# akanimax/thr3ed_atom

Measured on AMD Instinct MI355X. Metric: ray-samples/sec (fwd+bwd) training step, 800x800 images @ 128^3 SH-2 ReLU field, higher is better.
Workload: dtype f32

## Files before the change

### thr3ed_atom_amd/csrc/relu_field_kernels.hip

```cpp
#include "rf_device.h"

#include <atomic>

namespace {

#ifndef RF_FWD_WAVES
#define RF_FWD_WAVES 4
#endif
#ifndef RF_EMIT_WAVES
#define RF_EMIT_WAVES 6
#endif
#ifndef RF_EMIT_G
#define RF_EMIT_G 2
#endif
constexpr short kNoBrick = -1;

struct __attribute__((packed, aligned(4))) f4u {
  float v[4];
};
struct __attribute__((packed, aligned(4))) f3u {
  float v[3];
};
typedef float vf2 __attribute__((ext_vector_type(2)));
typedef float vf4 __attribute__((ext_vector_type(4)));
// ... 411 lines not shown
      }
      if (!L::kCorner && g.layout == RF_LAYOUT_SPLIT) {
        if constexpr (!L::kCorner) {
          const float rest = rest_colour_sums<K>(prod);
          if (has && ls.closes_colour) my_rgb[slot * 4 + ls.colour] = rest;
        }
      } else {
#pragma unroll
        for (int ch = 0; ch < 3; ++ch) rgb[ch] = group_sum_to_last<LPS>(rgb[ch]);
        if (has && sub == LPS - 1) {
          if constexpr (L::kCorner) {
#pragma unroll
            for (int ch = 0; ch < 3; ++ch) rgb[ch] = kC0 * rgb[ch];
          }
          my_rgb[slot * 4 + 0] = rgb[0];
          my_rgb[slot * 4 + 1] = rgb[1];
          my_rgb[slot * 4 + 2] = rgb[2];
        }
      }
    }
    wave_lds_fence();

    const float raw_r = fast_base ? fast_rgb[0] : (base_in_p0 ? fast_rgb[0] + my_rgb[slot * 4 + 0] : my_rgb[slot * 4 + 0]);
    const float raw_g = fast_base ? fast_rgb[1] : (base_in_p0 ? fast_rgb[1] + my_rgb[slot * 4 + 1] : my_rgb[slot * 4 + 1]);
    const float raw_b = fast_base ? fast_rgb[2] : (base_in_p0 ? fast_rgb[2] + my_rgb[slot * 4 + 2] : my_rgb[slot * 4 + 2]);
    if (need) {
      part_c[0] += w * sigmoidf_(raw_r);
      part_c[1] += w * sigmoidf_(raw_g);
      part_c[2] += w * sigmoidf_(raw_b);
    }
    if (sm.valid) {
      part_acc += w;
      part_depth += w * sm.z;
    }
    if constexpr (SAVE) {
      if (need) {
        const long long idx = ray * (long long)r.S + chunk * kWave + slot;
        float4 cv;
        cv.x = raw_r;
        cv.y = raw_g;
        cv.z = raw_b;
        cv.w = sigma;
        store_f4<RF_NT_CACHE_STORE>(reinterpret_cast<float4*>(out.cache) + idx, cv);
        if (RF_NT_CACHE_STORE)
          __builtin_nontemporal_store(T, out.tcache + idx);
        else
          out.tcache[idx] = T;
      }
      my_cmask = (lane == (chunk & (kWave - 1))) ? mask : my_cmask;
      if (out.hist) add_key_runs<false>(out.hist, need ? brick_key(sm.cell.i0, g, out.brick_shift, out.nby, out.nbz) : -1, lane);
    }
    wave_lds_fence();
    if (T_carry == 0.0f) break;
  }

  const float cr = wave_sum(part_c[0]), cg = wave_sum(part_c[1]), cb = wave_sum(part_c[2]);
  const float acc = wave_sum(part_acc), depth = wave_sum(part_depth);
  if (lane == 0) {
    const float bg = white ? (1.0f - acc) : 0.0f;
    out.colour[ray * 3 + 0] = white ? cr + bg : cr;
    out.colour[ray * 3 + 1] = white ? cg + bg : cg;
    out.colour[ray * 3 + 2] = white ? cb + bg : cb;
    out.depth[ray] = depth;
    out.acc[ray] = acc;
    const float q = depth / acc;
    out.disparity[ray] = 1.0f / ((q != q) ? q : fmaxf(kZeroPlus, q));
    if constexpr (SAVE) out.stop[ray] = processed;
  }
  if constexpr (SAVE) {
    flush_cmasks(cmask_group);
    for (int gq = cmask_group + 1; gq * kWave < nchunks; ++gq) flush_cmasks(gq);
  }
}

template <int K, bool DIFFUSE, bool SAVE>
__global__ __launch_bounds__(kBlock, RF_FWD_WAVES) void render_forward_kernel(GridArgs g, RayArgs r, OutArgs out, uint32_t flags) {
  __shared__ __attribute__((aligned(16))) uint32_t s_entry[kWavesPerBlock][kWave * kEntryFwd];
  __shared__ __attribute__((aligned(16))) float s_rgb[kWavesPerBlock][kWave * 4];
  const int lane = threadIdx.x & (kWave - 1);
  const int wave = __builtin_amdgcn_readfirstlane(threadIdx.x >> 6);
  render_forward_ray<K, DIFFUSE, SAVE>(g, r, out, flags, (long long)blockIdx.x * kWavesPerBlock + wave, lane, s_entry[wave], s_rgb[wave]);
}

struct ForwardPair {
  RayArgs r[2];
  OutArgs out[2];
  uint32_t flags[2];
};
__device__ __forceinline__ void fold_step_switches(GridArgs& g, RayArgs& r, uint32_t& flags) {
  g.layout = RF_LAYOUT_SPLIT;
  g.bricked = 0;
  g.near32 = 1;
  g.mode = RF_DENSITY_RELU;
  g.occ = nullptr;
  g.step[2] = 1u;
#pragma unroll
  for (int a = 0; a < 3; ++a) g.jump[a] = g.step[a];
  r.trand = nullptr;
  r.jitter = 1;
  r.cam = 0;
  r.H = r.W = 1;
  r.focal = 1.0f;
#pragma unroll
  for (int i = 0; i < 12; ++i) r.pose[i] = 0.0f;
  flags &= ~(uint32_t)(RF_FLAG_OCCUPANCY_SKIP | RF_FLAG_AABB_SAMPLING);
}

template <int K, bool DIFFUSE, bool STEP>
__device__ __forceinline__ void forward_pair_ray(const GridArgs& g, const RayArgs& r, const OutArgs& out, uint32_t flags, long long ray, int lane,
                                                 uint32_t* my_entry, float* my_rgb) {
  if constexpr (STEP) {
    GridArgs gl = g;
    RayArgs rl = r;
    fold_step_switches(gl, rl, flags);
    render_forward_ray<K, DIFFUSE, true>(gl, rl, out, flags, ray, lane, my_entry, my_rgb);
  } else {
    render_forward_ray<K, DIFFUSE, true>(g, r, out, flags, ray, lane, my_entry, my_rgb);
  }
}

template <int K, bool STEP>
__global__ __launch_bounds__(kBlock, RF_FWD_WAVES) void render_forward_pair_kernel(GridArgs g, ForwardPair p) {
  __shared__ __attribute__((aligned(16))) uint32_t s_entry[kWavesPerBlock][kWave * kEntryFwd];
  __shared__ __attribute__((aligned(16))) float s_rgb[kWavesPerBlock][kWave * 4];
  const int lane = threadIdx.x & (kWave - 1);
  const int wave = __builtin_amdgcn_readfirstlane(threadIdx.x >> 6);
  const long long ray = (long long)blockIdx.x * (kWavesPerBlock / 2) + (wave & 1);
  if (wave < 2) {
    if constexpr (K == 1)
      forward_pair_ray<1, true, STEP>(g, p.r[0], p.out[0], p.flags[0], ray, lane, s_entry[wave], s_rgb[wave]);
    else
      forward_pair_ray<K, false, STEP>(g, p.r[0], p.out[0], p.flags[0], ray, lane, s_entry[wave], s_rgb[wave]);
  } else {
    forward_pair_ray<1, true, STEP>(g, p.r[1], p.out[1], p.flags[1], ray, lane, s_entry[wave], s_rgb[wave]);
  }
}

#ifndef RF_TILE_WAVES
#define RF_TILE_WAVES 4
#endif
constexpr int kTileXS = 18;
constexpr int kTileSlots = (3 * kTileXS + 16 + 3) / 4 * 4;
#define RF_TILE_SLOT(lane) ((lane) + ((lane) >> 4) * (kTileXS - 16))
struct TileCell {
  int c0[3], e[3];
  float w[8];
};
__device__ __forceinline__ TileCell tile_cell(const Cell& c, const GridArgs& g) {
  const int dims3[3] = {g.X, g.Y, g.Z};
  TileCell t;
  float aw[3][2];
#pragma unroll
  for (int a = 0; a < 3; ++a) {
    const int i0 = c.i0[a];
    const bool ok0 = i0 >= 0, ok1 = i0 + 1 < dims3[a];
    t.c0[a] = max(i0, 0);
    t.e[a] = (ok0 && ok1) ? 1 : 0;
    aw[a][0] = ok0 ? c.w0[a] : 0.0f;
    aw[a][1] = ok1 ? c.w1[a] : 0.0f;
  }
  const float wxy[4] = {aw[0][0] * aw[1][0], aw[0][1] * aw[1][0], aw[0][0] * aw[1][1], aw[0][1] * aw[1][1]};
#pragma unroll
  for (int k = 0; k < 8; ++k) t.w[k] = wxy[k & 3] * aw[2][k >> 2];
  return t;
}

__device__ __forceinline__ void tile_window_origin(bool pending, unsigned long long pm, const int c0[3], int O[3]) {
  const int anchor = ((pm >> 27) & 1ull) ? 27 : __builtin_ctzll(pm);
#pragma unroll
  for (int a = 0; a < 3; ++a) {
    const int A = __builtin_amdgcn_readlane(c0[a], anchor);
    const bool below1 = __ballot(pending && c0[a] < A) != 0ull, below2 = __ballot(pending && c0[a] < A - 1) != 0ull;
    O[a] = A - (below1 ? 1 : 0) - (below2 ? 1 : 0);
  }
}

struct TileWindow {
  vf4 b, q0, q1, q2, q3, q4, q5;
};
__device__ __forceinline__ unsigned int tile_window_node(const GridArgs& g, const int O[3], int lane) {
  const int nx = min(O[0] + (lane >> 4), g.X - 1), ny = min(O[1] + ((lane >> 2) & 3), g.Y - 1), nz = min(O[2] + (lane & 3), g.Z - 1);
  return node_lin(g, nx, ny, nz);
}
__device__ __forceinline__ const char* tile_record(const float* tensor, long long stride, unsigned int lin, int near32) {
  if (near32) return reinterpret_cast<const char*>(tensor) + (size_t)__umul24(lin, (unsigned int)stride * 4u);
  return reinterpret_cast<const char*>(tensor + (size_t)lin * (size_t)stride);
}
__device__ __forceinline__ void tile_window_load_base(TileWindow& wdw, const GridArgs& g, unsigned int lin) {
  wdw.b = *reinterpret_cast<const vf4*>(tile_record(g.dens, g.dstride, lin, g.near32));
}
__device__ __forceinline__ void tile_window_load_rest(TileWindow& wdw, const GridArgs& g, unsigned int lin) {
  const char* rp = tile_record(g.feat, g.fstride, lin, g.near32);
  wdw.q0 = *reinterpret_cast<const vf4*>(rp);
  wdw.q1 = *reinterpret_cast<const vf4*>(rp + 16);
  wdw.q2 = *reinterpret_cast<const vf4*>(rp + 32);
  wdw.q3 = *reinterpret_cast<const vf4*>(rp + 48);
  wdw.q4 = *reinterpret_cast<const vf4*>(rp + 64);
  wdw.q5 = *reinterpret_cast<const vf4*>(rp + 80);
}
__device__ __forceinline__ void tile_window_store_rest(const TileWindow& wdw, vf4* my_rest, int lane) {
  vf4* d = my_rest + RF_TILE_SLOT(lane) * 6;
  d[0] = wdw.q0;
  d[1] = wdw.q1;
  d[2] = wdw.q2;
  d[3] = wdw.q3;
  d[4] = wdw.q4;
  d[5] = wdw.q5;
}

__device__ __forceinline__ bool tile_interpolate_base(bool pending, const TileCell& tc, const int O[3], const vf4* my_base, const GridArgs& g, float T, int nk[8],
                                                      float& sigma, float raw[3], bool& need) {
// ... 597 lines not shown
      dl[u] = sm.delta;
      ix[u][0] = sm.cell.idx[0];
      ix[u][1] = sm.cell.idx[1];
      ix[u][2] = sm.cell.idx[2];
      counted[u] = (cm[u] >> lane) & 1ull;
      const int key = counted[u] ? brick_key(sm.cell.i0, g, gr.brick_shift, gr.nby, gr.nbz) : -1;
      const bool active = key >= 0;
      const int prev = __shfl_up(key, 1);
      const bool head = active && (lane == 0 || prev != key);
      const unsigned long long heads = __ballot(head);
      const unsigned long long ends = __ballot(head || !active);
      const unsigned long long above = (lane == 63) ? 0ull : (ends & ~((2ull << lane) - 1ull));
      const int run = (above ? __builtin_ctzll(above) : 64) - lane;
      const unsigned long long below = heads & ((lane == 63) ? ~0ull : ((2ull << lane) - 1ull));
      hl_[u] = below ? 63 - __builtin_clzll(below) : 0;
      if (head) base_[u] = atomicAdd(&gr.cursor[key], run);
    }
#pragma unroll
    for (int u = 0; u < G; ++u) {
      if (cm[u] == 0ull) continue;
      const bool have = counted[u];
      const float sigma = have ? cv[u].w : 0.0f;
      const float T = have ? Tc[u] : 0.0f;
      float E;
      const float alpha = occupancy_alpha(sigma * dl[u], E);
      const float w = alpha * T;
      const float Tn = T * E;
      const float raw[3] = {cv[u].x, cv[u].y, cv[u].z};
      float c[3], e = gD * zz[u] + gA;
#pragma unroll
      for (int ch = 0; ch < 3; ++ch) {
        c[ch] = sigmoidf_(raw[ch]);
        e += gC[ch] * (c[ch] - white);
      }
      const float we = have ? w * e : 0.0f;
      const float incl = wave_incl_rscan_add(we, lane);
      const float after = (incl - we) + suffix;
      suffix += __shfl(incl, 0, kWave);
      const float g_sigma = dl[u] * (Tn * e - after);
      float g_pre = density_pre_grad(g_sigma, sigma, g.mode);
      const int pos = __shfl(base_[u], hl_[u]) + (lane - hl_[u]);
      if (have) {
        const float graw[3] = {(w * gC[0]) * (c[0] * (1.0f - c[0])), (w * gC[1]) * (c[1] * (1.0f - c[1])), (w * gC[2]) * (c[2] * (1.0f - c[2]))};
        float4* dst = gr.sorted + (long long)pos * QE;
        if constexpr (KE == 1) {
          store_f4<RF_NT_RECORD_STORE>(dst + 0, make_float4(ix[u][0], ix[u][1], ix[u][2], 0.0f));
          store_f4<RF_NT_RECORD_STORE>(dst + 1, make_float4(g_pre * g.rho, graw[0] * kC0, graw[1] * kC0, graw[2] * kC0));
        } else {
          store_f4<RF_NT_RECORD_STORE>(dst + 0, make_float4(ix[u][0], ix[u][1], ix[u][2], g_pre * g.rho));
          store_f4<RF_NT_RECORD_STORE>(dst + 1, make_float4(graw[0], graw[1], graw[2], vdir[0]));
          store_f4<RF_NT_RECORD_STORE>(dst + 2, make_float4(vdir[1], vdir[2], 0.0f, 0.0f));
        }
      }
    }
  }
}

template <int K, bool DIFFUSE>
__global__ __launch_bounds__(kBlock, RF_EMIT_WAVES) void render_emit_direct_kernel(GridArgs g, RayArgs r, OutArgs fwd, GradArgs gr, uint32_t flags) {
  const int lane = threadIdx.x & (kWave - 1);
  const int wave = __builtin_amdgcn_readfirstlane(threadIdx.x >> 6);
  render_emit_direct_ray<K, DIFFUSE>(g, r, fwd, gr, flags, (long long)blockIdx.x * kWavesPerBlock + wave, lane);
}

struct EmitPair {
  RayArgs r[2];
  OutArgs fwd[2];
  GradArgs gr[2];
  uint32_t flags[2];
};
template <int K, bool DIFFUSE, bool STEP>
__device__ __forceinline__ void emit_pair_ray(const GridArgs& g, const RayArgs& r, const OutArgs& fwd, const GradArgs& gr, uint32_t flags, long long ray, int lane) {
  if constexpr (STEP) {
    GridArgs gl = g;
    RayArgs rl = r;
    fold_step_switches(gl, rl, flags);
    render_emit_direct_ray<K, DIFFUSE>(gl, rl, fwd, gr, flags, ray, lane);
  } else {
    render_emit_direct_ray<K, DIFFUSE>(g, r, fwd, gr, flags, ray, lane);
  }
}

template <int K, bool STEP>
__global__ __launch_bounds__(kBlock, RF_EMIT_WAVES) void render_emit_direct_pair_kernel(GridArgs g, EmitPair p) {
  const int lane = threadIdx.x & (kWave - 1);
  const int wave = __builtin_amdgcn_readfirstlane(threadIdx.x >> 6);
  const long long ray = (long long)blockIdx.x * (kWavesPerBlock / 2) + (wave & 1);
  for (int i = 0; i < 2; ++i)
    if (p.gr[i].hist_clear)
      for (long long k = (long long)blockIdx.x * blockDim.x + threadIdx.x; k < p.gr[i].nkeys; k += (long long)gridDim.x * blockDim.x) p.gr[i].hist_clear[k] = 0;
  GradArgs gr = p.gr[wave < 2 ? 0 : 1];
  gr.hist_clear = nullptr;
  if (wave < 2) {
    if constexpr (K == 1)
      emit_pair_ray<1, true, STEP>(g, p.r[0], p.fwd[0], gr, p.flags[0], ray, lane);
    else
      emit_pair_ray<K, false, STEP>(g, p.r[0], p.fwd[0], gr, p.flags[0], ray, lane);
  } else {
    emit_pair_ray<1, true, STEP>(g, p.r[1], p.fwd[1], gr, p.flags[1], ray, lane);
  }
}

constexpr int kMaxListsPerKind = 8;
constexpr int kRangeEntries = 15;
constexpr int kMaxRangesKind = kRangeEntries * kMaxListsPerKind;

struct BrickList {
  const float4* rec;
  const long long* offsets;
};

__device__ __forceinline__ void adam_update(float& p, float& m, float& v, float g, float step, float b1, float b2, float eps,
                                            float inv_bc2_sqrt) {
  const float mm = m + (g - m) * (1.0f - b1);
  const float vv = v * b2 + (g * g) * (1.0f - b2);
  const float denom = __builtin_amdgcn_sqrtf(vv) * inv_bc2_sqrt + eps;
  p = p - step * (mm * __builtin_amdgcn_rcpf(denom));
  m = mm;
  v = vv;
}

struct AdamArgs {
  float* p1;
  float* p2;
  float* m1;
  float* m2;
  float* v1;
  float* v2;
  float step;
  float b1, b2, eps;
  float inv_bc2_sqrt;
  int byte_offsets_fit_32_bits;
};

struct BrickArgs {
  BrickList wide[kMaxListsPerKind];
  BrickList narrow[kMaxListsPerKind];
  int nwide, nnarrow;
  int shift;
  int nbx, nby, nbz;
  int brick_first;
  int accumulate;
  int fmul;
  int stagger;
  AdamArgs adam;
  int parts;
  float* partial;
  int* part_state;
};

template <int Q>
__global__ void expand_records_kernel(const float4* __restrict__ rec, const long long* __restrict__ perm,
                                      const long long* __restrict__ begin_ptr, long long capacity, float4* __restrict__ out) {
  const long long begin = *begin_ptr;
  const long long items = (capacity - begin) * Q;
  for (long long it = (long long)blockIdx.x * blockDim.x + threadIdx.x; it < items; it += (long long)gridDim.x * blockDim.x) {
    const long long i = begin + it / Q;
    const int part = (int)(it % Q);
    out[i * Q + part] = rec[perm[i] * Q + part];
  }
}

struct BinLists {
  const int* hist[2];
  long long* offsets[2];
  int* cursor[2];
};

__device__ __forceinline__ void bin_offsets_body(const BinLists& lists, int nkeys, int list, int block) {
  const int* __restrict__ hist = lists.hist[list];
  long long* __restrict__ offsets = lists.offsets[list];
  int* __restrict__ cursor = lists.cursor[list];
  __shared__ int s_front[16], s_own[16];
  const int t = threadIdx.x, lane = t & (kWave - 1), wave = t >> 6;
  const int seg0 = block * 1024;
  int front = 0;
// ... 1127 lines not shown
    if (ZERO_GRAD) gradp[i] = 0.0f;
  }
}

struct L1Sets {
  const float* colour[2];
  float* grad[2];
  float* sums[2];
};

__device__ __forceinline__ void l1_loss_grad_body(const L1Sets& sets, const float* __restrict__ target, long long n3, float gscale, int set,
                                                  int block, int nblocks) {
  const float* __restrict__ colour = sets.colour[set];
  float* __restrict__ grad = sets.grad[set];
  float* __restrict__ sums = sets.sums[set];
  float abs_sum = 0.0f, sq_sum = 0.0f;
  for (long long i = (long long)block * blockDim.x + threadIdx.x; i < n3; i += (long long)nblocks * blockDim.x) {
    const float d = colour[i] - target[i];
    abs_sum += fabsf(d);
    sq_sum += d * d;
    grad[i] = (d > 0.0f) ? gscale : ((d < 0.0f) ? -gscale : 0.0f);
  }
  __shared__ float s_part[2][16];
  abs_sum = wave_sum(abs_sum);
  sq_sum = wave_sum(sq_sum);
  const int wave = threadIdx.x >> 6;
  if ((threadIdx.x & (kWave - 1)) == 0) {
    s_part[0][wave] = abs_sum;
    s_part[1][wave] = sq_sum;
  }
  __syncthreads();
  if (threadIdx.x == 0) {
    float a = 0.0f, b = 0.0f;
    for (int w = 0; w < (int)(blockDim.x >> 6); ++w) {
      a += s_part[0][w];
      b += s_part[1][w];
    }
    unsafeAtomicAdd(sums + 0, a);
    unsafeAtomicAdd(sums + 1, b);
  }
}

__global__ void l1_loss_grad_kernel(L1Sets sets, const float* __restrict__ target, long long n3, float gscale) {
  l1_loss_grad_body(sets, target, n3, gscale, blockIdx.y, blockIdx.x, gridDim.x);
}

__global__ void l1_loss_pair_kernel(L1Sets sets, const float* __restrict__ target, long long n3, float gscale, float inv_n3, float* __restrict__ out) {
  l1_loss_grad_body(sets, target, n3, gscale, blockIdx.y, blockIdx.x, gridDim.x);
  if (threadIdx.x == 0) {
    float* ws = sets.sums[0];
    unsigned int* ticket = reinterpret_cast<unsigned int*>(ws + 4);
    __threadfence();
    const unsigned int total = gridDim.x * gridDim.y;
    if (atomicAdd(ticket, 1u) == total - 1u) {
      __threadfence();
      float v[4];
#pragma unroll
      for (int i = 0; i < 4; ++i) v[i] = atomicExch(ws + i, 0.0f);
      atomicExch(ticket, 0u);
      const float l0 = v[0] * inv_n3, l1 = v[2] * inv_n3;
      out[0] = l0 + l1;
      out[1] = l0;
      out[2] = v[1] * inv_n3;
      out[3] = l1;
      out[4] = v[3] * inv_n3;
    }
  }
}

__global__ __launch_bounds__(1024) void loss_and_offsets_kernel(L1Sets sets, const float* __restrict__ target, long long n3, float gscale,
                                                                int loss_blocks, BinLists lists, int nkeys, int offset_blocks, int passes) {
  if (!((passes >> (blockIdx.y & 1)) & 1)) return;
  if (blockIdx.y < 2) {
    if ((int)blockIdx.x < loss_blocks) l1_loss_grad_body(sets, target, n3, gscale, blockIdx.y, blockIdx.x, loss_blocks);
  } else if ((int)blockIdx.x < offset_blocks) {
    bin_offsets_body(lists, nkeys, blockIdx.y - 2, blockIdx.x);
  }
}

}

extern "C" {

#ifdef RF_BRICK_PROFILE
int rf_debug_brick_profile(unsigned long long* out_host, int reset) {
  if (hipDeviceSynchronize() != hipSuccess) return RF_ERR_LAUNCH;
  if (out_host && hipMemcpyFromSymbol(out_host, HIP_SYMBOL(g_brick_prof), sizeof(g_brick_prof)) != hipSuccess) return RF_ERR_LAUNCH;
  if (reset) {
    unsigned long long zero[8] = {};
    if (hipMemcpyToSymbol(HIP_SYMBOL(g_brick_prof), zero, sizeof(zero)) != hipSuccess) return RF_ERR_LAUNCH;
  }
  return RF_OK;
}
#endif

int rf_abi_version(void) { return RF_ABI_VERSION; }

int rf_abi_struct_size(int which) {
  switch (which) {
    case 0: return (int)sizeof(RFGrid);
    case 1: return (int)sizeof(RFRayBatch);
    case 2: return (int)sizeof(RFRenderOut);
    case 3: return (int)sizeof(RFRenderGrads);
    case 4: return (int)sizeof(RFBrickList);
    case 5: return (int)sizeof(RFAdamState);
    case 6: return (int)sizeof(RFCamera);
    case 7: return (int)sizeof(RFRaySelection);
    case 8: return (int)sizeof(RFPassScratch);
    case 9: return (int)sizeof(RFTrainStep);
    case 10: return (int)sizeof(RFGeometryOut);
    case 11: return (int)sizeof(RFImage);
    default: return -1;
  }
}

const char* rf_error_string(int code) {
  switch (code) {
    case RF_OK:
      return "ok";
    case RF_ERR_NULL_POINTER:
      return "null pointer";
    case RF_ERR_BAD_SHAPE:
      return "bad shape, size or stride";
    case RF_ERR_UNSUPPORTED:
      return "unsupported configuration (SH degree must be 0..3, density mode a RF_DENSITY_* value, brick size 4 or 8 -- 8 for SH degree 3 -- with at most 4096 bricks for 16-bit keys; the optimizer in the brick flush needs split storage and SH degree 0 or 2)";
    case RF_ERR_LAUNCH:
      return "HIP kernel launch failed";
    default:
      return "unknown error code";
  }
}

int rf_cast_rays(int32_t height, int32_t width, float focal, const float* rotation_host, const float* translation_host,
                 float* origins_dev, float* directions_dev, void* stream) {
  if (!rotation_host || !translation_host || !origins_dev || !directions_dev) return RF_ERR_NULL_POINTER;
  if (height < 1 || width < 1) return RF_ERR_BAD_SHAPE;
  Pose pose;
  for (int i = 0; i < 9; ++i) pose.r[i] = rotation_host[i];
  for (int i = 0; i < 3; ++i) pose.t[i] = translation_host[i];
  const long long n = (long long)height * width;
  hipLaunchKernelGGL(cast_rays_kernel, dim3(grid_1d(n, 256)), dim3(256), 0, (hipStream_t)stream, height, width, focal,
                     pose, origins_dev, directions_dev);
  return launch_status();
}

int rf_cast_selected_rays(int32_t height, int32_t width, float focal, const float* poses_dev, int32_t num_poses,
                          const int64_t* pixel_index_dev, int64_t num_rays, float* origins_dev, float* directions_dev,
                          void* stream) {
  if (num_rays == 0) return RF_OK;
  if (!poses_dev || !pixel_index_dev || !origins_dev || !directions_dev) return RF_ERR_NULL_POINTER;
  if (height < 1 || width < 1 || num_poses < 1 || num_rays < 0) return RF_ERR_BAD_SHAPE;
  hipLaunchKernelGGL(cast_selected_rays_kernel, dim3(grid_1d(num_rays, 256)), dim3(256), 0, (hipStream_t)stream, height,
                     width, focal, poses_dev, num_poses, pixel_index_dev, (long long)num_rays, origins_dev,
                     directions_dev);
  return launch_status();
}

static int select_impl(int32_t height, int32_t width, float focal, const float* poses_dev, const int64_t* image_ids_dev,
                       int32_t num_batch_images, const float* pixel_table_dev, uint64_t key, int64_t first_index, int64_t num_rays,
                       float* origins_dev, float* directions_dev, float* pixels_dev, int64_t* pixel_index_dev, float* zero4_dev,
                       void* stream) {
  if (num_rays == 0) return RF_OK;
  if (!poses_dev || !pixel_table_dev || !origins_dev || !directions_dev || !pixels_dev) return RF_ERR_NULL_POINTER;
  if (height < 1 || width < 1 || num_batch_images < 1 || num_rays < 0 || first_index < 0) return RF_ERR_BAD_SHAPE;
  const unsigned long long P = (unsigned long long)num_batch_images * height * width;
  if ((unsigned long long)(first_index + num_rays) > P) return RF_ERR_BAD_SHAPE;
// ... 122 lines not shown
  }
  const unsigned blocks = ray_blocks(rays->num_rays);
  hipStream_t st = (hipStream_t)stream;
  const bool diffuse = flags & RF_FLAG_RENDER_DIFFUSE;
  const int K = grid->num_features / 3;
  if (rays->camera && !save) {
    const bool tiles = !rays->t_rand_dev && rays->num_samples <= kTileMaxSamples && frame_uses_packets(grid, g, rays->camera, flags);
    if (tiles) {
      const int W = rays->camera->width;
      const int row0 = (int)(rays->first_ray / W), row1 = (int)((rays->first_ray + rays->num_rays - 1) / W);
      const int tile_rows = (row1 - row0) / 8 + 1, tiles_x = (W + 7) / 8;
      static const int wpb = env_int("RF_TILE_WPB", 1) == 4 ? 4 : 1;
      static const bool xcd_rows = env_flag("RF_TILE_XCD_ROWS", true);
      const int KT = diffuse ? 1 : K;
      auto launch = [&](auto k, auto waves, auto xr) {
        constexpr int WPB = decltype(waves)::value;
        const long long wgs = decltype(xr)::value ? (long long)((tile_rows + 7) / 8) * 8 * ((tiles_x + WPB - 1) / WPB) : ((long long)tile_rows * tiles_x + WPB - 1) / WPB;
        hipLaunchKernelGGL((render_frame_tile_kernel<decltype(k)::value, WPB, decltype(xr)::value>), dim3((unsigned)wgs), dim3(kWave * WPB), 0, st, g, r, o, flags, row0, tile_rows, tiles_x);
        return launch_status();
      };
      using One = std::integral_constant<int, 1>;
      using Four = std::integral_constant<int, 4>;
      if (KT == 4 || KT == 16)
        return dispatch_sh(KT, ShSet<4, 16>{}, [&](auto k) { return launch(k, One{}, std::true_type{}); });
      return dispatch_sh(KT, ShSet<9, 1>{}, [&](auto k) {
        if (wpb == 4) return xcd_rows ? launch(k, Four{}, std::true_type{}) : launch(k, Four{}, std::false_type{});
        return xcd_rows ? launch(k, One{}, std::true_type{}) : launch(k, One{}, std::false_type{});
      });
    }
  }
  return dispatch_render(K, diffuse, [&](auto k, auto d) {
    if (save)
      hipLaunchKernelGGL((render_forward_kernel<decltype(k)::value, decltype(d)::value, true>), dim3(blocks), dim3(kBlock), 0, st, g, r, o, flags);
    else
      hipLaunchKernelGGL((render_forward_kernel<decltype(k)::value, decltype(d)::value, false>), dim3(blocks), dim3(kBlock), 0, st, g, r, o, flags);
    return launch_status();
  });
}

static bool step_pair_specialised(const RFGrid* grid, const GridArgs& g, const RFRayBatch* const rays[2], const uint32_t flags[2]) {
  if (!(grid->layout == RF_LAYOUT_SPLIT && g.layout == RF_LAYOUT_SPLIT && !g.bricked && g.near32 && grid->density_mode == RF_DENSITY_RELU)) return false;
  for (int i = 0; i < 2; ++i) {
    if (rays[i]->camera || rays[i]->t_rand_dev || !(flags[i] & RF_FLAG_JITTER_KEYED)) return false;
    if (flags[i] & (RF_FLAG_OCCUPANCY_SKIP | RF_FLAG_AABB_SAMPLING)) return false;
  }
  return env_flag("RF_STEP_SPECIALISED", true);
}

int rf_step_kernel_specialised(const RFGrid* grid, const RFRayBatch* rays, const uint32_t* flags) {
  int rc = check_grid(grid);
  if (rc != RF_OK) return rc;
  if (!rays || !flags) return RF_ERR_NULL_POINTER;
  const RFRayBatch* const rr[2] = {&rays[0], &rays[1]};
  for (int i = 0; i < 2; ++i) {
    rc = check_rays(rr[i]);
    if (rc != RF_OK) return rc;
  }
  if (!renders_pair_up(rr, flags)) return RF_ERR_UNSUPPORTED;
  return step_pair_specialised(grid, to_args(grid), rr, flags) ? 1 : 0;
}

static int forward_pair_impl(const RFGrid* grid, const RFRayBatch* const rays[2], const uint32_t flags[2], const RFRenderOut* const outs[2], void* stream) {
  int rc = check_grid(grid);
  if (rc != RF_OK) return rc;
  ForwardPair p;
  for (int i = 0; i < 2; ++i) {
    rc = check_rays(rays[i]);
    if (rc != RF_OK) return rc;
    const RFRenderOut* out = outs[i];
    if (!out || !out->colour_dev || !out->depth_dev || !out->acc_dev || !out->disparity_dev) return RF_ERR_NULL_POINTER;
    if (!has_caches(out)) return RF_ERR_UNSUPPORTED;
    if ((flags[i] & RF_FLAG_OCCUPANCY_SKIP) && !grid->occupancy_dev) return RF_ERR_NULL_POINTER;
    p.r[i] = to_args(rays[i], flags[i]);
    p.out[i] = to_args(out);
    p.flags[i] = flags[i];
    if (out->key_hist_dev) {
      rc = set_key_hist(grid, out, &p.out[i]);
      if (rc != RF_OK) return rc;
    }
  }
  if (!renders_pair_up(rays, flags)) return RF_ERR_UNSUPPORTED;
  if (rays[0]->num_rays == 0) return RF_OK;
  const GridArgs g = to_args(grid);
  const unsigned blocks = (unsigned)((rays[0]->num_rays + 1) / 2);
  const bool specialised = step_pair_specialised(grid, g, rays, flags);
  return dispatch_sh(grid->num_features / 3, ShAll{}, [&](auto k) {
    if (specialised)
      hipLaunchKernelGGL((render_forward_pair_kernel<decltype(k)::value, true>), dim3(blocks), dim3(kBlock), 0, (hipStream_t)stream, g, p);
    else
      hipLaunchKernelGGL((render_forward_pair_kernel<decltype(k)::value, false>), dim3(blocks), dim3(kBlock), 0, (hipStream_t)stream, g, p);
    return launch_status();
  });
}

static int backward_impl(const RFGrid* grid, const RFRayBatch* rays, uint32_t flags, const RFRenderOut* fwd,
                         const RFRenderGrads* grads, GradArgs gr, void* stream) {
  int rc = check_grid(grid);
  if (rc != RF_OK) return rc;
  rc = check_rays(rays);
  if (rc != RF_OK) return rc;
  if (!fwd || !grads) return RF_ERR_NULL_POINTER;
  if (rays->num_rays == 0) return RF_OK;
  if (!has_caches(fwd)) return RF_ERR_NULL_POINTER;
  const GridArgs g = to_args(grid);
  const RayArgs r = to_args(rays, flags);
  const OutArgs o = to_args(fwd);
  set_grads(grads, &gr);
  const unsigned blocks = ray_blocks(rays->num_rays);
  hipStream_t st = (hipStream_t)stream;
  return dispatch_render(grid->num_features / 3, flags & RF_FLAG_RENDER_DIFFUSE, [&](auto k, auto d) {
    constexpr int K = decltype(k)::value;
    constexpr bool DIFFUSE = decltype(d)::value;
    if (gr.sorted)
      hipLaunchKernelGGL((render_emit_direct_kernel<K, DIFFUSE>), dim3(blocks), dim3(kBlock), 0, st, g, r, o, gr, flags);
    else if (gr.keys)
      hipLaunchKernelGGL((render_backward_kernel<K, DIFFUSE, 1>), dim3(blocks), dim3(kBlock), 0, st, g, r, o, gr, flags);
    else
      hipLaunchKernelGGL((render_backward_kernel<K, DIFFUSE, 0>), dim3(blocks), dim3(kBlock), 0, st, g, r, o, gr, flags);
    return launch_status();
  });
}

int rf_render_backward(const RFGrid* grid, const RFRayBatch* rays, uint32_t flags, const RFRenderOut* fwd,
                       const RFRenderGrads* grads, float* grad_densities_dev, float* grad_features_dev, void* stream) {
  if (!grad_densities_dev) return RF_ERR_NULL_POINTER;
  if (grid && !grad_features_dev && !second_tensor_optional(grid)) return RF_ERR_NULL_POINTER;
  GradArgs gr = {};
  gr.gdens = grad_densities_dev;
  gr.gfeat = grad_features_dev;
  return backward_impl(grid, rays, flags, fwd, grads, gr, stream);
}

int rf_render_backward_emit(const RFGrid* grid, const RFRayBatch* rays, uint32_t flags, const RFRenderOut* fwd,
                            const RFRenderGrads* grads, int32_t brick_size, int16_t* keys_dev, float* records_dev,
                            int32_t* hist_dev, void* stream) {
  if (!grid) return RF_ERR_NULL_POINTER;
  if (!keys_dev || !records_dev) return RF_ERR_NULL_POINTER;
  int shift, nb[3];
  const int rc = brick_geometry(grid, brick_size, &shift, nb, true);
  if (rc != RF_OK) return rc;
  GradArgs gr = {};
  gr.keys = keys_dev;
  gr.records = records_dev;
  gr.brick_shift = shift;
  gr.nby = nb[1];
  gr.nbz = nb[2];
  gr.hist = hist_dev;
  return backward_impl(grid, rays, flags, fwd, grads, gr, stream);
}

static int emit_pair_impl(const RFGrid* grid, const RFRayBatch* const rays[2], const uint32_t flags[2], const RFPassScratch* const pass[2], void* stream) {
  int rc = check_grid(grid);
  if (rc != RF_OK) return rc;
  EmitPair p;
  for (int i = 0; i < 2; ++i) {
    rc = check_rays(rays[i]);
    if (rc != RF_OK) return rc;
    const RFPassScratch& ps = *pass[i];
    const RFRenderOut* fwd = &ps.out;
    if (!ps.cursor_dev || !ps.records_sorted_dev || !ps.grad_colour_dev) return RF_ERR_NULL_POINTER;
    if (!has_caches(fwd)) return RF_ERR_NULL_POINTER;
    rc = emit_direct_args(grid, fwd->brick_size, ps.cursor_dev, ps.records_sorted_dev, fwd->key_hist_dev, &p.gr[i]);
    if (rc != RF_OK) return rc;
    p.gr[i].gcolour = ps.grad_colour_dev;
    p.r[i] = to_args(rays[i], flags[i]);
    p.fwd[i] = to_args(fwd);
    p.flags[i] = flags[i];
  }
  if (!renders_pair_up(rays, flags)) return RF_ERR_UNSUPPORTED;
  if (rays[0]->num_rays == 0) return RF_OK;
  const GridArgs g = to_args(grid);
  const unsigned blocks = (unsigned)((rays[0]->num_rays + 1) / 2);
  const bool specialised = step_pair_specialised(grid, g, rays, flags);
  return dispatch_sh(grid->num_features / 3, ShAll{}, [&](auto k) {
    if (specialised)
      hipLaunchKernelGGL((render_emit_direct_pair_kernel<decltype(k)::value, true>), dim3(blocks), dim3(kBlock), 0, (hipStream_t)stream, g, p);
    else
      hipLaunchKernelGGL((render_emit_direct_pair_kernel<decltype(k)::value, false>), dim3(blocks), dim3(kBlock), 0, (hipStream_t)stream, g, p);
    return launch_status();
  });
}

int rf_render_forward_pair(const RFGrid* grid, const RFRayBatch* rays, const uint32_t* flags, const RFRenderOut* outs, void* stream) {
  if (!grid || !rays || !flags || !outs) return RF_ERR_NULL_POINTER;
  const RFRayBatch* const rr[2] = {&rays[0], &rays[1]};
  const RFRenderOut* const oo[2] = {&outs[0], &outs[1]};
  if (rays[0].camera || rays[1].camera) return RF_ERR_UNSUPPORTED;
  return forward_pair_impl(grid, rr, flags, oo, stream);
}

int rf_render_backward_emit_direct_pair(const RFGrid* grid, const RFRayBatch* rays, const uint32_t* flags, const RFPassScratch* passes, void* stream) {
  if (!grid || !rays || !flags || !passes) return RF_ERR_NULL_POINTER;
  if (passes[0].out.brick_size != passes[1].out.brick_size) return RF_ERR_BAD_SHAPE;
  const RFRayBatch* const rr[2] = {&rays[0], &rays[1]};
  const RFPassScratch* const pp[2] = {&passes[0], &passes[1]};
  return emit_pair_impl(grid, rr, flags, pp, stream);
}

int rf_render_backward_emit_direct(const RFGrid* grid, const RFRayBatch* rays, uint32_t flags, const RFRenderOut* fwd,
                                   const RFRenderGrads* grads, int32_t brick_size, int32_t* cursor_dev,
                                   float* records_sorted_dev, int32_t* hist_clear_dev, void* stream) {
  if (!grid) return RF_ERR_NULL_POINTER;
  GradArgs gr;
  const int rc = emit_direct_args(grid, brick_size, cursor_dev, records_sorted_dev, hist_clear_dev, &gr);
  if (rc != RF_OK) return rc;
  return backward_impl(grid, rays, flags, fwd, grads, gr, stream);
}

extern "C++" {
template <int Q>
static int launch_expand(const float* records_dev, const int64_t* perm_dev, const int64_t* begin_dev, int64_t capacity, float* out, hipStream_t st) {
  hipLaunchKernelGGL((expand_records_kernel<Q>), dim3(grid_1d(capacity * Q, 256, 256LL * 16)), dim3(256), 0, st,
                     reinterpret_cast<const float4*>(records_dev), reinterpret_cast<const long long*>(perm_dev),
                     reinterpret_cast<const long long*>(begin_dev), (long long)capacity, reinterpret_cast<float4*>(out));
  return launch_status();
}
}

int rf_expand_records(const RFGrid* grid, const float* records_dev, const int64_t* perm_dev, const int64_t* begin_dev,
                      int64_t capacity, int32_t render_diffuse, float* records_sorted_dev, void* stream) {
  const int rc = check_grid(grid);
  if (rc != RF_OK) return rc;
  if (capacity == 0) return RF_OK;
  if (!records_dev || !perm_dev || !begin_dev || !records_sorted_dev) return RF_ERR_NULL_POINTER;
  if (capacity < 0) return RF_ERR_BAD_SHAPE;
  const int diffuse = render_diffuse || grid->num_features == 3;
  hipStream_t st = (hipStream_t)stream;
  if (diffuse) return launch_expand<2>(records_dev, perm_dev, begin_dev, capacity, records_sorted_dev, st);
  return launch_expand<3>(records_dev, perm_dev, begin_dev, capacity, records_sorted_dev, st);
}

static int bin_offsets_impl(const int32_t* const hist[2], int64_t* const offsets[2], int32_t* const cursor[2], int nlists, int32_t num_keys,
                            void* stream) {
  if (num_keys < 1 || num_keys > (1 << 21)) return RF_ERR_BAD_SHAPE;
  BinLists l = {};
  for (int i = 0; i < nlists; ++i) {
    if (!hist[i] || !offsets[i] || !cursor[i]) return RF_ERR_NULL_POINTER;
    l.hist[i] = hist[i];
    l.offsets[i] = reinterpret_cast<long long*>(offsets[i]);
    l.cursor[i] = cursor[i];
  }
  hipLaunchKernelGGL(bin_offsets_kernel, dim3((num_keys + 1023) / 1024, nlists), dim3(1024), 0, (hipStream_t)stream, l, num_keys);
  return launch_status();
}

int rf_bin_offsets_pair(const int32_t* const* hist_dev, int32_t num_keys, int64_t* const* offsets_dev, int32_t* const* cursor_dev, void* stream) {
  if (!hist_dev || !offsets_dev || !cursor_dev) return RF_ERR_NULL_POINTER;
  const int32_t* h[2] = {hist_dev[0], hist_dev[1]};
  int64_t* o[2] = {offsets_dev[0], offsets_dev[1]};
  int32_t* c[2] = {cursor_dev[0], cursor_dev[1]};
  return bin_offsets_impl(h, o, c, 2, num_keys, stream);
}

int rf_bin_offsets(const int32_t* hist_dev, int32_t num_keys, int64_t* offsets_dev, int32_t* cursor_dev, void* stream) {
  const int32_t* h[2] = {hist_dev, nullptr};
  int64_t* o[2] = {offsets_dev, nullptr};
  int32_t* c[2] = {cursor_dev, nullptr};
  return bin_offsets_impl(h, o, c, 1, num_keys, stream);
}

extern "C++" {
// ... 487 lines not shown
```

Measured before the change: 17.96 billion.

## Shrink pair kernels to one ray per block and pin diffuse args in SGPRs

New measurement: 18.08 billion, median of 6. About the same (+0.7%).

```diff
diff --git a/thr3ed_atom_amd/csrc/relu_field_kernels.hip b/thr3ed_atom_amd/csrc/relu_field_kernels.hip
--- a/thr3ed_atom_amd/csrc/relu_field_kernels.hip
+++ b/thr3ed_atom_amd/csrc/relu_field_kernels.hip
@@ -517,6 +517,20 @@
   render_forward_ray<K, DIFFUSE, SAVE>(g, r, out, flags, (long long)blockIdx.x * kWavesPerBlock + wave, lane, s_entry[wave], s_rgb[wave]);
 }
 
+#ifdef RF_PAIR_PROBE
+constexpr int kPairProbeWords = 8 * 256 * 4 * 2;
+__device__ unsigned int g_pair_probe[2][kPairProbeWords];
+__device__ __forceinline__ void pair_probe_count(int kernel, bool specular, int lane) {
+  const unsigned int hw = __builtin_amdgcn_s_getreg(((32 - 1) << 11) | 4);
+  const unsigned int xcc = __builtin_amdgcn_s_getreg(((4 - 1) << 11) | 20);
+  const unsigned int slot = ((((xcc & 7u) << 8) | ((hw >> 8) & 255u)) << 3) | (((hw >> 4) & 3u) << 1) | (specular ? 0u : 1u);
+  if (lane == 0) atomicAdd(&g_pair_probe[kernel][slot], 1u);
+}
+#define RF_PAIR_PROBE_COUNT(kernel, specular, lane) pair_probe_count(kernel, specular, lane)
+#else
+#define RF_PAIR_PROBE_COUNT(kernel, specular, lane) do { } while (0)
+#endif
+
 struct ForwardPair {
   RayArgs r[2];
   OutArgs out[2];
@@ -541,6 +555,11 @@
   flags &= ~(uint32_t)(RF_FLAG_OCCUPANCY_SKIP | RF_FLAG_AABB_SAMPLING);
 }
 
+template <typename V>
+__device__ __forceinline__ void hold_scalar(V& v) {
+  asm volatile("" : "+s"(v));
+}
+
 template <int K, bool DIFFUSE, bool STEP>
 __device__ __forceinline__ void forward_pair_ray(const GridArgs& g, const RayArgs& r, const OutArgs& out, uint32_t flags, long long ray, int lane,
                                                  uint32_t* my_entry, float* my_rgb) {
@@ -548,20 +567,42 @@
     GridArgs gl = g;
     RayArgs rl = r;
     fold_step_switches(gl, rl, flags);
-    render_forward_ray<K, DIFFUSE, true>(gl, rl, out, flags, ray, lane, my_entry, my_rgb);
+    if constexpr (DIFFUSE) {
+      OutArgs ol = out;
+      hold_scalar(ol.cache);
+      hold_scalar(ol.tcache);
+      hold_scalar(ol.hist);
+      hold_scalar(ol.brick_shift);
+      hold_scalar(ol.nby);
+      hold_scalar(ol.nbz);
+      hold_scalar(gl.step[0]);
+      hold_scalar(gl.step[1]);
+      render_forward_ray<K, DIFFUSE, true>(gl, rl, ol, flags, ray, lane, my_entry, my_rgb);
+    } else {
+      render_forward_ray<K, DIFFUSE, true>(gl, rl, out, flags, ray, lane, my_entry, my_rgb);
+    }
   } else {
     render_forward_ray<K, DIFFUSE, true>(g, r, out, flags, ray, lane, my_entry, my_rgb);
   }
 }
 
+#ifndef RF_FWD_PAIR_WAVES
+#define RF_FWD_PAIR_WAVES 2
+#endif
+#ifndef RF_EMIT_PAIR_WAVES
+#define RF_EMIT_PAIR_WAVES 2
+#endif
+static_assert((RF_FWD_PAIR_WAVES == 2 || RF_FWD_PAIR_WAVES == 4) && (RF_EMIT_PAIR_WAVES == 2 || RF_EMIT_PAIR_WAVES == 4), "one or two rays per block");
+constexpr int kFwdPairRays = RF_FWD_PAIR_WAVES / 2, kEmitPairRays = RF_EMIT_PAIR_WAVES / 2;
 template <int K, bool STEP>
-__global__ __launch_bounds__(kBlock, RF_FWD_WAVES) void render_forward_pair_kernel(GridArgs g, ForwardPair p) {
-  __shared__ __attribute__((aligned(16))) uint32_t s_entry[kWavesPerBlock][kWave * kEntryFwd];
-  __shared__ __attribute__((aligned(16))) float s_rgb[kWavesPerBlock][kWave * 4];
+__global__ __launch_bounds__(kWave * RF_FWD_PAIR_WAVES, RF_FWD_WAVES) void render_forward_pair_kernel(GridArgs g, ForwardPair p) {
+  __shared__ __attribute__((aligned(16))) uint32_t s_entry[RF_FWD_PAIR_WAVES][kWave * kEntryFwd];
+  __shared__ __attribute__((aligned(16))) float s_rgb[RF_FWD_PAIR_WAVES][kWave * 4];
   const int lane = threadIdx.x & (kWave - 1);
   const int wave = __builtin_amdgcn_readfirstlane(threadIdx.x >> 6);
-  const long long ray = (long long)blockIdx.x * (kWavesPerBlock / 2) + (wave & 1);
-  if (wave < 2) {
+  const long long ray = (long long)blockIdx.x * kFwdPairRays + (wave % kFwdPairRays);
+  RF_PAIR_PROBE_COUNT(0, wave < kFwdPairRays, lane);
+  if (wave < kFwdPairRays) {
     if constexpr (K == 1)
       forward_pair_ray<1, true, STEP>(g, p.r[0], p.out[0], p.flags[0], ray, lane, s_entry[wave], s_rgb[wave]);
     else
@@ -1325,16 +1366,17 @@
 }
 
 template <int K, bool STEP>
-__global__ __launch_bounds__(kBlock, RF_EMIT_WAVES) void render_emit_direct_pair_kernel(GridArgs g, EmitPair p) {
+__global__ __launch_bounds__(kWave * RF_EMIT_PAIR_WAVES, RF_EMIT_WAVES) void render_emit_direct_pair_kernel(GridArgs g, EmitPair p) {
   const int lane = threadIdx.x & (kWave - 1);
   const int wave = __builtin_amdgcn_readfirstlane(threadIdx.x >> 6);
-  const long long ray = (long long)blockIdx.x * (kWavesPerBlock / 2) + (wave & 1);
+  const long long ray = (long long)blockIdx.x * kEmitPairRays + (wave % kEmitPairRays);
   for (int i = 0; i < 2; ++i)
     if (p.gr[i].hist_clear)
       for (long long k = (long long)blockIdx.x * blockDim.x + threadIdx.x; k < p.gr[i].nkeys; k += (long long)gridDim.x * blockDim.x) p.gr[i].hist_clear[k] = 0;
-  GradArgs gr = p.gr[wave < 2 ? 0 : 1];
+  RF_PAIR_PROBE_COUNT(1, wave < kEmitPairRays, lane);
+  GradArgs gr = p.gr[wave < kEmitPairRays ? 0 : 1];
   gr.hist_clear = nullptr;
-  if (wave < 2) {
+  if (wave < kEmitPairRays) {
     if constexpr (K == 1)
       emit_pair_ray<1, true, STEP>(g, p.r[0], p.fwd[0], gr, p.flags[0], ray, lane);
     else
@@ -2628,6 +2670,19 @@
 
 extern "C" {
 
+#ifdef RF_PAIR_PROBE
+int rf_debug_pair_probe(unsigned int* out_host, int reset) {
+  if (hipDeviceSynchronize() != hipSuccess) return RF_ERR_LAUNCH;
+  if (out_host && hipMemcpyFromSymbol(out_host, HIP_SYMBOL(g_pair_probe), sizeof(g_pair_probe)) != hipSuccess) return RF_ERR_LAUNCH;
+  if (reset) {
+    void* table = nullptr;
+    if (hipGetSymbolAddress(&table, HIP_SYMBOL(g_pair_probe)) != hipSuccess || hipMemset(table, 0, sizeof(g_pair_probe)) != hipSuccess) return RF_ERR_LAUNCH;
+    if (hipDeviceSynchronize() != hipSuccess) return RF_ERR_LAUNCH;
+  }
+  return RF_OK;
+}
+#endif
+
 #ifdef RF_BRICK_PROFILE
 int rf_debug_brick_profile(unsigned long long* out_host, int reset) {
   if (hipDeviceSynchronize() != hipSuccess) return RF_ERR_LAUNCH;
@@ -2916,13 +2971,13 @@
   if (!renders_pair_up(rays, flags)) return RF_ERR_UNSUPPORTED;
   if (rays[0]->num_rays == 0) return RF_OK;
   const GridArgs g = to_args(grid);
-  const unsigned blocks = (unsigned)((rays[0]->num_rays + 1) / 2);
+  const unsigned blocks = (unsigned)((rays[0]->num_rays + kFwdPairRays - 1) / kFwdPairRays);
   const bool specialised = step_pair_specialised(grid, g, rays, flags);
   return dispatch_sh(grid->num_features / 3, ShAll{}, [&](auto k) {
     if (specialised)
-      hipLaunchKernelGGL((render_forward_pair_kernel<decltype(k)::value, true>), dim3(blocks), dim3(kBlock), 0, (hipStream_t)stream, g, p);
+      hipLaunchKernelGGL((render_forward_pair_kernel<decltype(k)::value, true>), dim3(blocks), dim3(kWave * RF_FWD_PAIR_WAVES), 0, (hipStream_t)stream, g, p);
     else
-      hipLaunchKernelGGL((render_forward_pair_kernel<decltype(k)::value, false>), dim3(blocks), dim3(kBlock), 0, (hipStream_t)stream, g, p);
+      hipLaunchKernelGGL((render_forward_pair_kernel<decltype(k)::value, false>), dim3(blocks), dim3(kWave * RF_FWD_PAIR_WAVES), 0, (hipStream_t)stream, g, p);
     return launch_status();
   });
 }
@@ -3004,13 +3059,13 @@
   if (!renders_pair_up(rays, flags)) return RF_ERR_UNSUPPORTED;
   if (rays[0]->num_rays == 0) return RF_OK;
   const GridArgs g = to_args(grid);
-  const unsigned blocks = (unsigned)((rays[0]->num_rays + 1) / 2);
+  const unsigned blocks = (unsigned)((rays[0]->num_rays + kEmitPairRays - 1) / kEmitPairRays);
   const bool specialised = step_pair_specialised(grid, g, rays, flags);
   return dispatch_sh(grid->num_features / 3, ShAll{}, [&](auto k) {
     if (specialised)
-      hipLaunchKernelGGL((render_emit_direct_pair_kernel<decltype(k)::value, true>), dim3(blocks), dim3(kBlock), 0, (hipStream_t)stream, g, p);
+      hipLaunchKernelGGL((render_emit_direct_pair_kernel<decltype(k)::value, true>), dim3(blocks), dim3(kWave * RF_EMIT_PAIR_WAVES), 0, (hipStream_t)stream, g, p);
     else
-      hipLaunchKernelGGL((render_emit_direct_pair_kernel<decltype(k)::value, false>), dim3(blocks), dim3(kBlock), 0, (hipStream_t)stream, g, p);
+      hipLaunchKernelGGL((render_emit_direct_pair_kernel<decltype(k)::value, false>), dim3(blocks), dim3(kWave * RF_EMIT_PAIR_WAVES), 0, (hipStream_t)stream, g, p);
     return launch_status();
   });
 }
```
